# cg-tuwien/StatMC

Hardware: AMD Instinct MI355X
Metric: denoised_mpixels_per_s (higher is better)
Workload: dtype f32

## Files before the change

### include/statmc_debug.h

```cpp
#ifndef STATMC_DEBUG_H
#define STATMC_DEBUG_H

#include "statmc.h"

#include <stddef.h>
#ifdef __cplusplus
extern "C" {
#endif

int statmc_debug_force_filter_variant(int variant);
int statmc_debug_force_filter_parts(int parts);
int statmc_debug_last_filter_parts(void);
int statmc_debug_last_filter_tail(int *parts_hi, int *tail_rows);

int statmc_debug_accumulate_resident_blocks(int n);
int statmc_debug_last_accumulate_grid(void);
int statmc_debug_accumulate_dma(int on);
int statmc_debug_accumulate_launch(int grid_mode, int dma_first);
int statmc_debug_accumulate_umul(int umul);
int statmc_debug_accumulate_tiles_variant(int umul, int order, int wg_per_cu);

int statmc_debug_accumulate_records_phases(int phases);

int statmc_debug_interference_probe(const void *stream_ptr, size_t stream_bytes, void *rmw_ptr, size_t rmw_bytes, float *ms);
int statmc_debug_placement_role(const void *ptr);
float statmc_debug_placement_fast_level(const float *probes_ms, int n, float self_ms);

int statmc_debug_welch_far_items(void);
int statmc_debug_last_workspace(void **ptr, size_t *bytes);

#ifdef __cplusplus
}
#endif
#endif
```

### statmc_amd/api.py

```python
import ctypes as C
import os

from . import build as _build

_HERE = os.path.dirname(os.path.abspath(__file__))

STATMC_OK = 0
ERR_INVALID, ERR_UNSUPPORTED, ERR_HIP, ERR_NO_DEVICE = -1, -2, -3, -4
DOF_PIXEL, DOF_WELCH = 0, 1
MAX_BUFFERS, MAX_GBUFFERS = 16, 8


class StatmcError(RuntimeError):
    def __init__(self, code, msg):
        super().__init__("statmc error %d: %s" % (code, msg))
        self.code = code


class Image(C.Structure):
    _fields_ = [("data", C.c_void_p), ("step", C.c_size_t), ("cols", C.c_int32), ("rows", C.c_int32)]


class FilterArgs(C.Structure):
    _fields_ = [
# ... 107 lines not shown
    lib.statmc_placement_info.argtypes = [C.POINTER(PlacementInfo)]
    lib.statmc_malloc_host.argtypes = [C.POINTER(C.c_void_p), C.c_size_t]
    lib.statmc_free_host.argtypes = [C.c_void_p]
    lib.statmc_memset.argtypes = [C.c_void_p, C.c_int, C.c_size_t, C.c_void_p]
    lib.statmc_upload.argtypes = [C.c_void_p, C.c_void_p, C.c_size_t, C.c_void_p]
    lib.statmc_download.argtypes = [C.c_void_p, C.c_void_p, C.c_size_t, C.c_void_p]
    lib.statmc_stream_create.argtypes = [C.POINTER(C.c_void_p)]
    lib.statmc_stream_create_with_priority.argtypes = [C.POINTER(C.c_void_p), C.c_int]
    lib.statmc_stream_destroy.argtypes = [C.c_void_p]
    lib.statmc_event_create.argtypes = [C.POINTER(C.c_void_p)]
    lib.statmc_event_destroy.argtypes = [C.c_void_p]
    lib.statmc_event_record.argtypes = [C.c_void_p, C.c_void_p]
    lib.statmc_stream_wait_event.argtypes = [C.c_void_p, C.c_void_p]
    lib.statmc_synchronize.argtypes = [C.c_void_p]
    lib.statmc_filter_f32.argtypes = [C.POINTER(FilterArgs)]
    lib.statmc_filter_f32x3.argtypes = [C.POINTER(FilterArgs)]
    lib.statmc_prepass.argtypes = [C.POINTER(FilterArgs), C.c_int]
    lib.statmc_window_filter.argtypes = [C.POINTER(FilterArgs), C.c_int]
    lib.statmc_pack_filter_inputs.argtypes = [C.POINTER(FilterArgs), C.POINTER(Image), C.c_int, C.c_int]
    lib.statmc_prepass_pack.argtypes = [C.POINTER(FilterArgs), C.POINTER(Image), C.c_int, C.c_int]
    lib.statmc_prepass_pack_rows.argtypes = [C.POINTER(FilterArgs), C.POINTER(Image), C.c_int, C.c_int, C.POINTER(C.c_int32), C.c_int]
    lib.statmc_halo_exchange.argtypes = [C.c_void_p, C.c_int, C.c_int, C.c_int, C.c_int, C.c_int]
    lib.statmc_halo_exchange_rccl.argtypes = [C.c_void_p, C.c_int, C.c_int, C.c_int, C.c_int, C.c_int, C.c_void_p, C.c_int]
    lib.statmc_rccl_unique_id.argtypes = [C.c_void_p]
    lib.statmc_rccl_comm_create.argtypes = [C.POINTER(C.c_void_p), C.c_int, C.c_int, C.c_void_p]
    lib.statmc_rccl_comm_destroy.argtypes = [C.c_void_p]
    lib.statmc_copy_rect.argtypes = [C.POINTER(Image), C.c_int, C.c_int, C.c_int, C.POINTER(Image), C.c_int, C.c_int, C.c_int,
                                     C.c_int, C.c_int, C.c_int, C.c_void_p]
    lib.statmc_set_device.argtypes = [C.c_int]
    lib.statmc_calculate_mean_vars.argtypes = [C.c_uint8, C.c_uint16, C.c_uint16, C.c_int,
                                               C.POINTER(Image), C.POINTER(Image), C.POINTER(Image),
                                               C.c_int, C.c_void_p]
    lib.statmc_accumulate.argtypes = [C.c_uint16, C.c_uint16, C.POINTER(StatType), C.c_int, C.c_void_p]
    lib.statmc_accumulate_rows.argtypes = [C.c_uint16, C.c_uint16, C.POINTER(StatType), C.c_int, C.c_int, C.c_int, C.c_void_p]
    lib.statmc_accumulate_row_ranges.argtypes = [C.c_uint16, C.c_uint16, C.POINTER(StatType), C.c_int, C.POINTER(C.c_int32), C.c_int, C.c_void_p]
    lib.statmc_accumulate_tiles.argtypes = [C.c_uint16, C.c_uint16, C.POINTER(StatType), C.c_int, C.c_void_p, C.c_void_p,
                                            C.c_void_p, C.c_int, C.c_void_p]
    lib.statmc_accumulate_records.argtypes = [C.c_uint16, C.c_uint16, C.POINTER(StatType), C.c_int, C.c_void_p, C.c_int64, C.c_void_p]
    lib.statmc_debug_accumulate_records_phases.argtypes = [C.c_int]
    lib.statmc_get_prepass_context.argtypes = [C.POINTER(PrepassContext)]
    lib.statmc_combine_statistics.argtypes = [C.c_uint16, C.c_uint16, C.POINTER(CombineEntry), C.c_int, C.c_void_p]
    lib.statmc_combine_many.argtypes = [C.c_uint16, C.c_uint16, C.POINTER(CombineManyEntry), C.c_int, C.c_int, C.c_void_p]
    lib.statmc_merge_tiles.argtypes = [C.c_uint16, C.c_uint16, C.c_int, C.c_int, C.c_void_p, C.c_void_p,
                                       C.c_void_p, C.c_int, C.c_int] + [C.c_void_p] * 6 + [C.c_void_p]
    lib.statmc_tile_moments.argtypes = [C.c_uint16, C.c_uint16, C.c_int, C.c_void_p, C.c_int,
                                        C.c_void_p, C.c_void_p]
    lib.statmc_film_update.argtypes = [C.c_void_p, C.c_size_t, C.c_float, C.c_float, C.c_void_p, C.c_void_p]
    lib.statmc_clock_probe.argtypes = [C.c_void_p, C.c_int, C.c_void_p]
    lib.statmc_debug_force_filter_variant.argtypes = [C.c_int]
    lib.statmc_debug_force_filter_parts.argtypes = [C.c_int]
    lib.statmc_debug_last_filter_parts.restype = C.c_int
    lib.statmc_debug_accumulate_resident_blocks.argtypes = [C.c_int]
    lib.statmc_debug_accumulate_dma.argtypes = [C.c_int]
    _lib = lib
    return lib


def check(rc):
    if rc != STATMC_OK:
        raise StatmcError(rc, load().statmc_last_error().decode())
    return rc


_setup_done = set()


def setup(device=0):
    if device not in _setup_done:
        check(load().statmc_setup(int(device)))
        _setup_done.add(device)


def set_filter_spec(spec=None, **fields):
    if spec is None and not fields:
        check(load().statmc_reset_filter_spec())
        return
    spec = spec if spec is not None else FilterSpec(**fields)
    check(load().statmc_set_filter_spec(C.byref(spec)))


def get_significance():
    return int(load().statmc_get_significance())


def get_filter_spec():
    spec = FilterSpec()
    check(load().statmc_get_filter_spec(C.byref(spec)))
    return spec


def last_filter_variant():
    return load().statmc_last_filter_variant().decode()


def force_filter_variant(v):
    check(load().statmc_debug_force_filter_variant(int(v)))


def accumulate_resident_blocks(n):
    check(load().statmc_debug_accumulate_resident_blocks(int(n)))


def accumulate_dma(on):
    check(load().statmc_debug_accumulate_dma(int(on)))


def force_filter_parts(k):
    check(load().statmc_set_filter_split(int(k)))


def set_filter_split(parts):
    check(load().statmc_set_filter_split(int(parts)))


def get_filter_split():
    return int(load().statmc_get_filter_split())


def filter_split_auto(width, height, radius):
    k = int(load().statmc_filter_split_auto(int(width), int(height), int(radius)))
    if k < 0:
        check(k)
    return k


def _torch():
    import torch
    return torch


def current_stream_handle():
    return C.c_void_p(_torch().cuda.current_stream().cuda_stream)


def image_of(t):
    assert t.is_cuda and t.element_size() == 4
    h, w = t.shape[0], t.shape[1]
    c = t.shape[2] if t.dim() == 3 else 1
    inner = (t.stride(1) == c and t.stride(2) == 1) if t.dim() == 3 else t.stride(1) == 1
    assert inner and t.stride(0) >= w * c, "device images must have packed pixels and a row pitch of at least one row"
    return Image(C.c_void_p(t.data_ptr()), t.stride(0) * 4, w, h)


def _img_array(tensors):
    arr = (Image * max(len(tensors), 1))()
    for i, t in enumerate(tensors):
        arr[i] = image_of(t)
    return arr


def make_filter_args(n, mean, m2, m3, film, mean_corr, disc, film_filtered, g_buffers, g_sds=None,
                     g_dr=None, filter_sd=10.0, radius=20, denoise_film=False, film_buffer=None,
                     film_filtered_buffer=None, roi=None, stream=None, keep=None, packed=None, film_origin=None,
                     packed_g_channels=None):
    tables = [mean_corr, mean, film, film_filtered, n]
    nb = max(len(t) for t in tables) if packed is None else 1
    ref = next(t[0] for t in tables if t) if packed is None else packed
# ... 315 lines not shown
```

### statmc_amd/csrc/statmc_abi.hip

```cpp

#include <algorithm>
#include <cmath>
#include <stdarg.h>
#include <stdio.h>
#include <string.h>

#include <memory>
#include <mutex>
#include <unordered_map>
#include <vector>

#include "statmc_device.h"

#include <atomic>

#include "t_quantiles.h"
#include "../../include/statmc_pinned_spec.h"

namespace {

thread_local char g_err[512] = "";
thread_local char g_variant[96] = "none";
thread_local int g_last_parts = 0, g_last_parts_hi = 0, g_last_tail_rows = 0;
thread_local const int *g_last_redo = nullptr;
thread_local int g_last_redo_n = 0;
std::mutex g_mu;

struct DeviceState {
    bool ready = false;
    int alpha_index = STATMC_PINNED_SIGNIFICANCE;
    statmc_filter_spec spec = STATMC_PINNED_SPEC;
    int cus = 0;
    int split = 0;
    int force_variant = 0;
    int acc_resident_blocks = 0, acc_umul = 1, acc_dma = 1;
    int acc_grid_mode = -1, acc_dma_first = 0;
    int rec_phases = 3;
    int tiles_umul = 2, tiles_order = 2, tiles_wg_per_cu = 0;
};
std::unordered_map<int, DeviceState> g_dev;

DeviceState current_state(int *dev_out = nullptr) {
    int dev = 0;
    if (hipGetDevice(&dev) != hipSuccess) return DeviceState();
    if (dev_out) *dev_out = dev;
    std::lock_guard<std::mutex> lk(g_mu);
    auto it = g_dev.find(dev);
    return it == g_dev.end() ? DeviceState() : it->second;
}

int fail(int code, const char *fmt, ...) {
    va_list ap;
    va_start(ap, fmt);
    vsnprintf(g_err, sizeof(g_err), fmt, ap);
    va_end(ap);
    return code;
}

}
namespace statmc {
int abi_fail(int code, const char *fmt, ...) {
    va_list ap;
    va_start(ap, fmt);
    vsnprintf(g_err, sizeof(g_err), fmt, ap);
    va_end(ap);
    return code;
}
}
namespace {

#define HIP_TRY(expr)                                                                          \
    do {                                                                                       \
        hipError_t e_ = (expr);                                                                \
        if (e_ != hipSuccess) return fail(STATMC_ERR_HIP, "%s: %s", #expr, hipGetErrorString(e_)); \
    } while (0)

#define NEED_READY()                                                                                      \
    const DeviceState dstate = current_state();                                                           \
    do {                                                                                                  \
        if (!dstate.ready)                                                                                \
            return fail(STATMC_ERR_NO_DEVICE, "statmc_setup() has not been called for the current device"); \
    } while (0)

inline hipStream_t S(void *s) { return reinterpret_cast<hipStream_t>(s); }

struct TabKey {
    int dev, r;
    float ds;
    bool operator==(const TabKey &o) const { return dev == o.dev && r == o.r && memcmp(&ds, &o.ds, 4) == 0; }
// ... 1023 lines not shown
    out->t_table = table;
    out->flags = (dstate.spec.dof == STATMC_DOF_WELCH ? 1 : 0) | (dstate.spec.small_n == STATMC_SMALL_N_EXCLUDE ? 2 : 0);
    out->reserved = 0;
    return STATMC_OK;
}

int statmc_accumulate(uint16_t width, uint16_t height, const statmc_stat_type *types, int n_types, void *stream) {
    return statmc_accumulate_rows(width, height, types, n_types, 0, height, stream);
}
int statmc_accumulate_rows(uint16_t width, uint16_t height, const statmc_stat_type *types, int n_types, int y0, int y1, void *stream) {
    const int32_t range[2] = {y0, y1};
    return statmc_accumulate_row_ranges(width, height, types, n_types, range, 1, stream);
}
int statmc_accumulate_row_ranges(uint16_t width, uint16_t height, const statmc_stat_type *types, int n_types, const int32_t *ranges,
                                 int n_ranges, void *stream) {
    NEED_READY();
    if (width == 0 || height == 0) return fail(STATMC_ERR_INVALID, "empty image");
    if (n_types < 0 || n_ranges < 0 || (long long)n_types * n_ranges > statmc::kMaxStatTypes)
        return fail(STATMC_ERR_INVALID, "stat types x row ranges must be in [0,%d]", statmc::kMaxStatTypes);
    if (n_types == 0 || n_ranges == 0) return STATMC_OK;
    if (!types || !ranges) return fail(STATMC_ERR_INVALID, "null types or ranges");
    statmc::AccumulateArgs k;
    memset(&k, 0, sizeof(k));
    k.n_types = 0;
    for (int r = 0; r < n_ranges; r++) {
        const int y0 = ranges[2 * r], y1 = ranges[2 * r + 1];
        if (y0 < 0 || y1 > height || y0 > y1) return fail(STATMC_ERR_INVALID, "rows [%d,%d) outside the %d-row image", y0, y1, (int)height);
        for (int q = 0; q < r; q++)
            if (y0 < ranges[2 * q + 1] && ranges[2 * q] < y1) return fail(STATMC_ERR_INVALID, "row ranges %d and %d overlap", q, r);
        if (y0 == y1) continue;
        for (int i = 0; i < n_types; i++) {
            statmc::AccumulateType &d = k.t[k.n_types];
            if (int rc = fill_stat_type(dstate, types[i], i, width, height, true, d)) return rc;
            const long long px0 = (long long)y0 * width, e0 = px0 * d.channels;
            if (d.samples) d.samples += e0;
            d.n += px0;
            d.mean += e0;
            if (d.m2) d.m2 += e0;
            if (d.m3) d.m3 += e0;
            if (d.film_mean) d.film_mean += e0;
            if (d.film_m2) d.film_m2 += e0;
            if (d.mean_corr) { d.mean_corr += e0; d.disc += e0; }
            d.n_elems = (long long)(y1 - y0) * width * d.channels;
            k.n_types++;
        }
    }
    if (k.n_types == 0) return STATMC_OK;
    k.resident_blocks = dstate.acc_resident_blocks;
    k.cus = dstate.cus;
    k.umul = dstate.acc_umul;
    k.dma = dstate.acc_dma;
    k.grid_mode = dstate.acc_grid_mode;
    k.dma_first = dstate.acc_dma_first;
    k.occ = 0;
    k.apart = 1;
    for (int i = 0; i < k.n_types && k.apart; i++)
        k.apart = statmc::placement_role_of(k.t[i].samples) == STATMC_MEM_STREAM && statmc::placement_role_of(k.t[i].mean) == STATMC_MEM_STATE;
    HIP_TRY(statmc::launch_accumulate(k, S(stream)));
    return STATMC_OK;
}

static bool aligned16(const void *p) { return (reinterpret_cast<uintptr_t>(p) & 15) == 0; }

static int fill_combine_entry(const DeviceState &ds, const statmc_combine_entry *entries, int n_entries, int i,
                              statmc::CombineEntry &k) {
    const statmc_combine_entry &e = entries[i];
    const statmc_stat_type &d = e.dst, &s = e.src;
    if (d.channels != 1 && d.channels != 3) return fail(STATMC_ERR_INVALID, "entries[%d]: channels must be 1 or 3", i);
    if (d.max_moment < 1 || d.max_moment > 3) return fail(STATMC_ERR_INVALID, "entries[%d]: max_moment must be 1..3", i);
    if (s.channels != d.channels || s.max_moment != d.max_moment)
        return fail(STATMC_ERR_INVALID, "entries[%d]: dst and src disagree on channels or max_moment", i);
    if (e.count_of == -1) {
        if (!d.n || !s.n) return fail(STATMC_ERR_INVALID, "entries[%d]: null n (count_of = -1: the entry's own counts)", i);
        if (d.n == s.n) return fail(STATMC_ERR_INVALID, "entries[%d]: dst.n is src.n", i);
        for (int j = 0; j < i; j++)
            if (entries[j].count_of == -1 && entries[j].dst.n == d.n)
                return fail(STATMC_ERR_INVALID, "entries[%d] and [%d] own the same count image", j, i);
    } else if (e.count_of < 0 || e.count_of >= n_entries || e.count_of == i || entries[e.count_of].count_of != -1) {
        return fail(STATMC_ERR_INVALID, "entries[%d]: bad count_of %d (-1, or an entry with counts of its own)", i, e.count_of);
    } else if (d.n || s.n) {
        return fail(STATMC_ERR_INVALID, "entries[%d]: borrows entry %d's counts, dst.n and src.n must be NULL", i, e.count_of);
    }
    const float *dp[statmc::kCombFields] = {d.mean, d.max_moment >= 2 ? d.m2 : nullptr, d.max_moment >= 3 ? d.m3 : nullptr,
                                            nullptr, nullptr};
    const float *sp[statmc::kCombFields] = {s.mean, s.max_moment >= 2 ? s.m2 : nullptr, s.max_moment >= 3 ? s.m3 : nullptr,
                                            nullptr, nullptr};
    static const char *names[statmc::kCombFields] = {"mean", "m2", "m3", "film_mean", "film_m2"};
    const bool film_mean = d.film_mean && d.film_mean != d.mean;
    const bool film_m2 = d.film_m2 && d.film_m2 != d.m2;
    if (film_m2 && !film_mean) return fail(STATMC_ERR_INVALID, "entries[%d]: film_m2 without a film_mean of its own", i);
    if (film_mean) {
        dp[statmc::kCombFilmMean] = d.film_mean;
        sp[statmc::kCombFilmMean] = s.film_mean;
    }
    if (film_m2) {
        dp[statmc::kCombFilmM2] = d.film_m2;
        sp[statmc::kCombFilmM2] = s.film_m2;
    }
    const int want = d.max_moment;
    for (int f = 0; f < statmc::kCombFields; f++) {
        const bool needed = f < want || (f == statmc::kCombFilmMean && film_mean) || (f == statmc::kCombFilmM2 && film_m2);
        if (!needed) continue;
        if (!dp[f] || !sp[f]) return fail(STATMC_ERR_INVALID, "entries[%d]: null %s", i, names[f]);
        if (dp[f] == sp[f]) return fail(STATMC_ERR_INVALID, "entries[%d]: dst.%s is src.%s", i, names[f], names[f]);
    }
    k.cnt_dst = e.count_of == -1 ? d.n : entries[e.count_of].dst.n;
// ... 229 lines not shown
                              (width + tile_size - 1) / tile_size, (height + tile_size - 1) / tile_size};
    HIP_TRY(statmc::launch_tile_moments(k, S(stream)));
    return STATMC_OK;
}

int statmc_clock_probe(int64_t *out, int cycles, void *stream) {
    NEED_READY();
    if (!out) return fail(STATMC_ERR_INVALID, "null out");
    if (cycles < 1 || cycles > (1 << 24)) return fail(STATMC_ERR_INVALID, "cycles must be in 1 .. 2^24");
    hipLaunchKernelGGL(clock_probe_kernel, dim3(1), dim3(64), 0, S(stream), reinterpret_cast<long long *>(out), (long long)cycles);
    HIP_TRY(hipGetLastError());
    return STATMC_OK;
}

int statmc_set_filter_split(int parts) {
    if (parts < 0 || parts > 64) return fail(STATMC_ERR_INVALID, "parts must be 0 (automatic) .. 64");
    int dev = 0;
    NEED_READY();
    HIP_TRY(hipGetDevice(&dev));
    std::lock_guard<std::mutex> lk(g_mu);
    g_dev[dev].split = parts;
    return STATMC_OK;
}
int statmc_get_filter_split(void) { return current_state().split; }
int statmc_filter_split_auto(int width, int height, int radius) {
    NEED_READY();
    if (width < 1 || height < 1 || radius < 1 || radius > 20) return fail(STATMC_ERR_INVALID, "need a non-empty image and a radius in 1..20");
    statmc::FilterArgs k;
    memset(&k, 0, sizeof(k));
    k.width = width;
    k.height = height;
    k.radius = radius;
    return statmc::whole_image_parts(k, true, dstate.cus, 0);
}

#define STATMC_DEBUG_SET(stmt)                                       \
    do {                                                             \
        int dev = 0;                                                 \
        NEED_READY();                                                \
        HIP_TRY(hipGetDevice(&dev));                                 \
        std::lock_guard<std::mutex> lk(g_mu);                        \
        DeviceState &d = g_dev[dev];                                 \
        stmt;                                                        \
        return STATMC_OK;                                            \
    } while (0)
int statmc_debug_force_filter_variant(int v) {
    if (v < 0 || v > 3) return fail(STATMC_ERR_INVALID, "statmc_debug_force_filter_variant(%d): 0 .. 3", v);
    STATMC_DEBUG_SET(d.force_variant = v);
}
int statmc_debug_accumulate_resident_blocks(int n) {
    STATMC_DEBUG_SET(d.acc_resident_blocks = n < 0 ? -1 : n);
}
int statmc_debug_last_accumulate_grid(void) { return (int)statmc::last_accumulate_grid(); }
int statmc_debug_accumulate_dma(int on) {
    if (on != 0 && on != 1) return fail(STATMC_ERR_INVALID, "statmc_debug_accumulate_dma(%d): 0 or 1", on);
    STATMC_DEBUG_SET(d.acc_dma = on);
}
int statmc_debug_accumulate_launch(int grid_mode, int dma_first) {
    STATMC_DEBUG_SET(d.acc_grid_mode = grid_mode < 0 ? -1 : grid_mode == 1 ? 1 : 0; d.acc_dma_first = dma_first ? 1 : 0);
}
int statmc_debug_accumulate_umul(int umul) {
    STATMC_DEBUG_SET(d.acc_umul = umul == 2 ? 2 : 1);
}
int statmc_debug_accumulate_tiles_variant(int umul, int order, int wg_per_cu) {
    STATMC_DEBUG_SET(d.tiles_umul = umul == 2 ? 2 : 1; d.tiles_order = order < 0 || order > 2 ? 0 : order; d.tiles_wg_per_cu = wg_per_cu < 0 ? 0 : wg_per_cu);
}
int statmc_debug_accumulate_records_phases(int phases) {
    if (phases < 1 || phases > 3) return fail(STATMC_ERR_INVALID, "statmc_debug_accumulate_records_phases(%d): 1, 2 or 3", phases);
    STATMC_DEBUG_SET(d.rec_phases = phases);
}
int statmc_debug_force_filter_parts(int k) { return statmc_set_filter_split(k < 0 ? 0 : k); }
int statmc_debug_last_filter_parts(void) { return g_last_parts; }
int statmc_debug_last_filter_tail(int *parts_hi, int *tail_rows) {
    if (parts_hi) *parts_hi = g_last_parts_hi;
    if (tail_rows) *tail_rows = g_last_tail_rows;
    return STATMC_OK;
}
int statmc_debug_welch_far_items(void) {
    if (g_last_redo == nullptr || g_last_redo_n <= 0) return -1;
    if (hipDeviceSynchronize() != hipSuccess) return -1;
    std::vector<int> f((size_t)g_last_redo_n);
    if (hipMemcpy(f.data(), g_last_redo, f.size() * sizeof(int), hipMemcpyDeviceToHost) != hipSuccess) return -1;
    int n = 0;
    for (int v : f) n += v != 0;
    return n;
}
int statmc_debug_last_workspace(void **ptr, size_t *bytes) {
    int dev = 0;
    HIP_TRY(hipGetDevice(&dev));
    std::lock_guard<std::mutex> lk(g_mu);
    *ptr = nullptr;
    *bytes = 0;
    for (auto &kv : g_ws)
        if (kv.first.dev == dev && kv.second.bytes > *bytes) {
            *ptr = kv.second.ptr;
            *bytes = kv.second.bytes;
        }
    return STATMC_OK;
}
}
```

### statmc_amd/csrc/statmc_device.h

```cpp
#pragma once

#include <hip/hip_runtime.h>
#include <stdint.h>

#include "../../include/statmc.h"

namespace statmc {

struct PrepassArgs {
    const int32_t *n;
    const float *mean, *m2, *m3;
    float *mean_corr, *disc;
    long long n_elems;
    int channels;
    int table;
    int welch;
    int small_n_exclude;
};

struct MeanVarsArgs {
    const int32_t *n;
    const float *film_m2;
    float *film_var;
    int width, height, channels, row_n_quirk;
};

constexpr int kMaxStatTypes = 16;
struct AccumulateType {
    const float *samples;
    int32_t *n;
    float *mean, *m2, *m3, *film_mean, *film_m2;
    long long n_elems;
    long long stride;
    int channels, n_samples, transform, max_moment;
    float *mean_corr, *disc;
    int pre_table;
    int pre_flags;
};
constexpr int kMaxSlots = 64;
struct AccumulateArgs {
    AccumulateType t[kMaxStatTypes];
    int n_types;
    int resident_blocks;
    int cus;
    int umul;
    int dma;
    int grid_mode;
    int dma_first;
    int occ;
    int apart;
    int n_slots;
    int type_slots[kMaxStatTypes];
    unsigned char slot_type[kMaxSlots], slot_rank[kMaxSlots];
};

struct AccumulateTilesArgs {
    AccumulateType t[kMaxStatTypes];
    int n_types;
    const int32_t *tile_bounds;
    const long long *tile_offsets;
    const int32_t *tile_samples;
    int n_tiles, width, height, vec;
    int dma;
    int umul, order, wg_per_cu;
    int dma_first;
};

enum { kCombMean = 0, kCombM2, kCombM3, kCombFilmMean, kCombFilmM2, kCombFields };
struct CombineEntry {
    int32_t *cnt_dst;
    const int32_t *cnt_src;
    float *d[kCombFields];
    const float *s[kCombFields];
    float *mean_corr, *disc;
    int channels, write_n, pre_table, pre_flags;
};
struct CombineArgs {
    CombineEntry e[kMaxStatTypes];
    int n_entries;
    int vec;
    long long n_px;
};
hipError_t launch_combine(const CombineArgs &a, hipStream_t s);

enum { kCombManyPlanes = 3, kCombManySrcPtrs = 1 + kCombManyPlanes, kCombManySlots = 90 };
struct CombineManyEntry {
    int32_t *cnt_dst;
    float *d[kCombManyPlanes];
    float *mean_corr, *disc;
    int channels, moments, write_n, pre;
};
struct CombineManyArgs {
    long long n_px;
    int n_entries, n_sources;
    int vec;
    int reserved;
    CombineManyEntry e[kMaxStatTypes];
    const void *src[kCombManySlots * kCombManySrcPtrs];
};
static_assert(sizeof(CombineManyArgs) <= 4096, "CombineManyArgs is passed by value: the kernel-argument limit");
hipError_t launch_combine_many(const CombineManyArgs &a, hipStream_t s);

struct RecordsArgs {
    statmc_stat_type t[kMaxStatTypes];
    statmc_prepass_context ctx;
    const int32_t *order;
// ... 58 lines not shown
    const int32_t *f_n[3];
    float *f_out[3];
    int f_active;
    const float *packed;
    int packed_ch;
    struct SymGeom {
        int tx0, ty0, ntx, nty;
        int fx0, fy0;
        long long item_stride4;
        float4 *patch;
        int pair;
        float *pair_images;
        float4 *border_extra;
        int *redo;
        int parts_hi, split_ty, n_lo_tiles, n_lo_items;
        int steps;
        const float *tab_rt;
        int g8;
        const float *rgb[2], *sc[2];
        float rgb_scale[2], sc_scale[2];
    } sym;
};

struct PackArgs {
    const float *mean_corr, *disc, *colour, *g0, *g1;
    float *packed;
    int src_w, src_h, dst_w, dst_x0, dst_y0;
    const float *s0, *s1;
    int ch;
    const int32_t *n;
};
hipError_t launch_pack_inputs(const PackArgs &a, hipStream_t s);

struct PrepassPackArgs {
    const int32_t *n;
    const float *mean, *m2, *m3, *colour, *g0, *g1;
    float *mean_corr, *disc;
    float *packed;
    int src_w, src_h, dst_w, dst_x0, dst_y0, table, welch, small_n_exclude;
    int split_row, skip_rows;
    const float *s0, *s1;
    int ch;
};
hipError_t launch_prepass_pack(const PrepassPackArgs &a, hipStream_t s);

hipError_t upload_t_tables();
hipError_t upload_t_table(int table, const float *host_4096);
const float *t_table_device_ptr(int table);
const float *t_table_sq_device_ptr(int table);
hipError_t launch_prepass(const PrepassArgs &a, hipStream_t s);
hipError_t launch_mean_vars(const MeanVarsArgs &a, hipStream_t s);
hipError_t launch_accumulate(const AccumulateArgs &a, hipStream_t s);
unsigned last_accumulate_grid();
hipError_t launch_accumulate_tiles(const AccumulateTilesArgs &a, hipStream_t s);
hipError_t launch_merge_tiles(const MergeTilesArgs &a, int n_tiles, int max_tile_pixels, hipStream_t s);
hipError_t launch_tile_moments(const TileMomentsArgs &a, hipStream_t s);
hipError_t launch_film_update(const void *pixels, long long n, float splat_scale, float scale, float *rgb, hipStream_t s);

enum { kFilterGeneric, kFilterLds, kFilterSym };
struct FilterPlan {
    int kernel;
    bool lds_r20;
    int per_launch;
    bool lds_tail;
    bool spatial_tab, sym_rt_tab;
    size_t partial_floats, patch_floats, image_floats, extra_floats, redo_floats;
    int redo_items;
    int tail_rows;
    char variant[48], tail_variant[96];
};
int plan_window_filter(FilterArgs &k, int channels, int n_buffers, int n_cus, int force_variant, int split, FilterPlan &p);
hipError_t launch_window_filter(const FilterPlan &p, bool tail, const FilterArgs &a, int channels, hipStream_t s);
int whole_image_parts(const FilterArgs &a, bool sym, int n_cus, int split);
size_t spatial_table_floats(int radius);
size_t sym_rt_table_floats(int radius);
void fill_sym_rt_table(float *host_tab, int radius, float ds);
void fill_spatial_table(float *host_tab, int radius, float ds);

int abi_fail(int code, const char *fmt, ...);
int placement_role_of(const void *ptr);
int placement_free(void *ptr);
hipError_t workspace_alloc(void **p, size_t bytes);
hipError_t workspace_free(void *p);
hipError_t placement_grant_peer(int owner_device, int peer_device);

}
```

### statmc_amd/csrc/statmc_pointwise.hip

```cpp

#include <type_traits>

#include "statmc_device.h"

#include "../../include/statmc_device_api.hpp"
#include "t_quantiles.h"

namespace statmc {

using device::CombineCounts;
using device::ElemState;
using device::add_sample;
using device::div_by_count;
using device::prepass_elem;
using device::refined_rcp;

constexpr int kAccURgbT = 3, kAccURgb = 3, kAccUF = 6;
constexpr int kAccPairGroup = 3;
constexpr int kAccWaves = 2;
constexpr int kAccDmaD = 3;
constexpr int kAccTilesDmaD = 3;
constexpr int acc_ring_floats(int d) { return d * 3 * 256; }
constexpr size_t acc_lds_bytes(int d) { return (size_t)4 * acc_ring_floats(d) * sizeof(float); }
template <int N> __device__ __forceinline__ void acc_wait_vmcnt() { asm volatile("s_waitcnt vmcnt(%0)" ::"n"(N) : "memory"); }
// ... 447 lines not shown
        const int n_active = left >= 64 ? 64 : left > 0 ? (int)left : 0;
        if (n_active > 0)
            accumulate_lane<C, MAXM, TRANSFORM, (!TRANSFORM && MAXM == 1) ? UMUL : 1, DMA>(t, p0, t.samples + p0 * C, t.stride, t.n_samples,
                                                                                            ring, active, n_active, dma_first);
        if (!active && g < n_groups) {
            for (long long p = p0; p < n_px && p < p0 + 4; p++)
                accumulate_pixel<C, MAXM, TRANSFORM>(t, p, t.samples + p * C, t.stride, t.n_samples);
        }
    }
}

template <int C, bool VEC, int UMUL, int DMA>
__device__ __forceinline__ void accumulate_dispatch(const AccumulateType &t, long long blk, long long nblk, float *ring, bool dma_first) {
    if (t.transform) {
        if (t.max_moment >= 3) accumulate_type<C, 3, true, VEC, UMUL, DMA>(t, blk, nblk, ring, dma_first);
        else if (t.max_moment == 2) accumulate_type<C, 2, true, VEC, UMUL, DMA>(t, blk, nblk, ring, dma_first);
        else accumulate_type<C, 1, true, VEC, UMUL, DMA>(t, blk, nblk, ring, dma_first);
    } else {
        if (t.max_moment >= 3) accumulate_type<C, 3, false, VEC, UMUL, DMA>(t, blk, nblk, ring, dma_first);
        else if (t.max_moment == 2) accumulate_type<C, 2, false, VEC, UMUL, DMA>(t, blk, nblk, ring, dma_first);
        else accumulate_type<C, 1, false, VEC, UMUL, DMA>(t, blk, nblk, ring, dma_first);
    }
}

template <bool VEC, int UMUL, int DMA, int OCC = kAccWaves>
__global__ __launch_bounds__(kBlock, OCC) void accumulate_kernel(AccumulateArgs a) {
    extern __shared__ __attribute__((aligned(16))) float acc_lds[];
    float *ring = DMA ? acc_lds + (threadIdx.x >> 6) * acc_ring_floats(DMA) : nullptr;
    if (a.resident_blocks > 0) {
        for (int i = 0; i < a.n_types; i++) {
            const AccumulateType t = a.t[((int)blockIdx.x + i) % a.n_types];
            if (t.channels == 3) accumulate_dispatch<3, VEC, UMUL, DMA>(t, blockIdx.x, gridDim.x, ring, a.dma_first != 0);
            else accumulate_dispatch<1, VEC, UMUL, DMA>(t, blockIdx.x, gridDim.x, ring, a.dma_first != 0);
        }
        return;
    }
    if (a.grid_mode == 1) {
        const int ti = blockIdx.x % a.n_types;
        const AccumulateType t = a.t[ti];
        const long long blk = blockIdx.x / a.n_types, nblk = gridDim.x / a.n_types;
        if (t.channels == 3) accumulate_dispatch<3, VEC, UMUL, DMA>(t, blk, nblk, ring, a.dma_first != 0);
        else accumulate_dispatch<1, VEC, UMUL, DMA>(t, blk, nblk, ring, a.dma_first != 0);
        return;
    }
    const int slot = blockIdx.x % a.n_slots, round = blockIdx.x / a.n_slots, n_rounds = gridDim.x / a.n_slots;
    const int ti = a.slot_type[slot];
    const AccumulateType t = a.t[ti];
    const long long blk = (long long)round * a.type_slots[ti] + a.slot_rank[slot];
    const long long nblk = (long long)n_rounds * a.type_slots[ti];
    if (t.channels == 3) accumulate_dispatch<3, VEC, UMUL, DMA>(t, blk, nblk, ring, a.dma_first != 0);
    else accumulate_dispatch<1, VEC, UMUL, DMA>(t, blk, nblk, ring, a.dma_first != 0);
}

static thread_local unsigned g_last_acc_grid = 0;
unsigned last_accumulate_grid() { return g_last_acc_grid; }

hipError_t launch_accumulate(const AccumulateArgs &a_in, hipStream_t s) {
    AccumulateArgs a = a_in;
    a.n_slots = 0;
    for (int i = 0; i < a.n_types; i++) {
        int w = a.t[i].channels * (a.t[i].transform ? 4 : 3);
        w = (w + 2) / 3;
        if (w < 1) w = 1;
        a.type_slots[i] = w;
        for (int r = 0; r < w && a.n_slots < kMaxSlots; r++) {
            a.slot_type[a.n_slots] = (unsigned char)i;
            a.slot_rank[a.n_slots] = (unsigned char)r;
            a.n_slots++;
        }
    }
    {
        unsigned char st[kMaxSlots], sr[kMaxSlots];
        int n = 0;
        for (int r = 0; n < a.n_slots; r++)
            for (int i = 0; i < a.n_types; i++)
                if (r < a.type_slots[i]) { st[n] = (unsigned char)i; sr[n] = (unsigned char)r; n++; }
        for (int k = 0; k < a.n_slots; k++) { a.slot_type[k] = st[k]; a.slot_rank[k] = sr[k]; }
    }
    bool vec = true;
    long long max_groups = 1;
    for (int i = 0; i < a.n_types; i++) {
        const AccumulateType &t = a.t[i];
        vec = vec && aligned16(t.samples) && aligned16(t.n) && aligned16(t.mean) &&
              (t.max_moment < 2 || aligned16(t.m2)) && (t.max_moment < 3 || aligned16(t.m3)) &&
              (!t.transform || (aligned16(t.film_mean) && aligned16(t.film_m2))) &&
              (!t.mean_corr || (aligned16(t.mean_corr) && aligned16(t.disc))) &&
              (t.n_elems % 4 == 0) && (t.stride % 4 == 0);
        const long long groups = (t.n_elems / t.channels + 3) / 4;
        if (groups > max_groups) max_groups = groups;
    }
    const int rounds = (grid_for(max_groups, 256 * 8) * a.n_types + a.n_slots - 1) / a.n_slots;
    const long long units = (max_groups + kBlock - 1) / kBlock;
    int max_s = 0;
    for (int i = 0; i < a.n_types; i++) max_s = a.t[i].n_samples > max_s ? a.t[i].n_samples : max_s;
    if (a.resident_blocks == 0 && a.grid_mode < 0 && a.apart && a.cus > 0 && max_s >= 256 && max_groups >= (1 << 18) && max_groups < 3 * (1 << 18)) {
        const double walks = (double)max_groups / ((double)a.cus * kBlock);
        if (walks / ceil(walks) >= 0.97) a.resident_blocks = a.cus;
    }
    if (a.resident_blocks < 0) a.resident_blocks = 0;
    if (a.grid_mode < 0) {
        const bool big = max_groups >= (1 << 20);
        if (a.apart) a.grid_mode = (max_s <= 16 || big || max_s >= 128) ? 1 : 0;
        else a.grid_mode = (max_s <= 8 || (max_s <= 16 && !big)) ? 1 : 0;
    }
    const dim3 grid(a.resident_blocks > 0 ? a.resident_blocks : a.grid_mode == 1 ? (unsigned)(units * a.n_types) : rounds * a.n_slots);
    g_last_acc_grid = grid.x;
    if (vec && a.dma) {
        hipLaunchKernelGGL((accumulate_kernel<true, 1, kAccDmaD>), grid, dim3(kBlock), acc_lds_bytes(kAccDmaD), s, a);
        return hipGetLastError();
    }
    if (vec && a.umul == 2)
        hipLaunchKernelGGL((accumulate_kernel<true, 2, 0>), grid, dim3(kBlock), 0, s, a);
    else if (vec)
        hipLaunchKernelGGL((accumulate_kernel<true, 1, 0>), grid, dim3(kBlock), 0, s, a);
    else
        hipLaunchKernelGGL((accumulate_kernel<false, 1, 0>), grid, dim3(kBlock), 0, s, a);
    return hipGetLastError();
}

template <int C, int MAXM, bool TRANSFORM, int UMUL, int DMA>
__device__ __forceinline__ void accumulate_tile(const AccumulateType &t, const AccumulateTilesArgs &a, int x0, int y0,
                                                int tw, int th, long long off, int S, float *ring) {
    const int lane = threadIdx.x & 63;
    const int npx = tw * th;
    const float *base = t.samples + off * C;
    const long long stride = (long long)npx * C;
    const bool fast = a.vec && ((tw | x0 | a.width) & 3) == 0 && (off & 3) == 0;
    if (fast) {
        const int n_g = npx >> 2;
        for (int gw = 0; gw < n_g; gw += 64) {
            const int g = gw + lane;
            const bool active = g < n_g;
            const int i = g << 2, row = i / tw, col = i - row * tw;
            const long long p0 = (long long)(y0 + row) * a.width + x0 + col;
            accumulate_lane<C, MAXM, TRANSFORM, (!TRANSFORM && MAXM == 1) ? UMUL : 1, DMA>(t, p0, base + (long long)i * C, stride, S, ring, active,
                                                                                            n_g - gw >= 64 ? 64 : n_g - gw, a.dma_first != 0);
        }
    } else {
        for (int i = lane; i < npx; i += 64) {
            const int row = i / tw, col = i - row * tw;
            const long long p = (long long)(y0 + row) * a.width + x0 + col;
            accumulate_pixel<C, MAXM, TRANSFORM>(t, p, base + (long long)i * C, stride, S);
        }
    }
}

template <int C, int UMUL, int DMA>
__device__ __forceinline__ void accumulate_tile_dispatch(const AccumulateType &t, const AccumulateTilesArgs &a, int x0,
                                                         int y0, int tw, int th, long long off, int S, float *ring) {
    if (t.transform) {
        if (t.max_moment >= 3) accumulate_tile<C, 3, true, UMUL, DMA>(t, a, x0, y0, tw, th, off, S, ring);
        else if (t.max_moment == 2) accumulate_tile<C, 2, true, UMUL, DMA>(t, a, x0, y0, tw, th, off, S, ring);
// ... 479 lines not shown
```

Baseline: 388.5.

## Fuse radiance and feature-buffer accumulation into one persistent LDS-ring kernel

Adds a fused accumulate kernel that walks the radiance type and up to two RGB and two scalar feature types in one wave loop. It streams samples of all types into a shared LDS ring via global_load_lds with counted vmcnt waits, and keeps per-pixel state in registers across samples. Waves whose per-pixel counts differ fall back to a ragged per-type path. The kernel is launched with one block per CU when the shape heuristic matches (many samples, mid-size images) or when forced. It aims to cut per-type launch and slot overhead and overlap loads across types, at the cost of a large LDS footprint, single-block occupancy and high register pressure.

Result: faster. 393.4, median of 6 (+1.3%).

```diff
diff --git a/include/statmc_debug.h b/include/statmc_debug.h
--- a/include/statmc_debug.h
+++ b/include/statmc_debug.h
@@ -15,6 +15,8 @@
 
 int statmc_debug_accumulate_resident_blocks(int n);
 int statmc_debug_last_accumulate_grid(void);
+int statmc_debug_accumulate_fused(int mode);
+int statmc_debug_last_accumulate_fused(void);
 int statmc_debug_accumulate_dma(int on);
 int statmc_debug_accumulate_launch(int grid_mode, int dma_first);
 int statmc_debug_accumulate_umul(int umul);
diff --git a/statmc_amd/api.py b/statmc_amd/api.py
--- a/statmc_amd/api.py
+++ b/statmc_amd/api.py
@@ -183,6 +183,8 @@
     lib.statmc_debug_last_filter_parts.restype = C.c_int
     lib.statmc_debug_accumulate_resident_blocks.argtypes = [C.c_int]
     lib.statmc_debug_accumulate_dma.argtypes = [C.c_int]
+    lib.statmc_debug_accumulate_fused.argtypes = [C.c_int]
+    lib.statmc_debug_last_accumulate_fused.restype = C.c_int
     _lib = lib
     return lib
 
@@ -234,6 +236,14 @@
 
 def accumulate_dma(on):
     check(load().statmc_debug_accumulate_dma(int(on)))
+
+
+def accumulate_fused(mode):
+    check(load().statmc_debug_accumulate_fused(int(mode)))
+
+
+def last_accumulate_fused():
+    return int(load().statmc_debug_last_accumulate_fused())
 
 
 def force_filter_parts(k):
diff --git a/statmc_amd/csrc/statmc_abi.hip b/statmc_amd/csrc/statmc_abi.hip
--- a/statmc_amd/csrc/statmc_abi.hip
+++ b/statmc_amd/csrc/statmc_abi.hip
@@ -35,6 +35,7 @@
     int force_variant = 0;
     int acc_resident_blocks = 0, acc_umul = 1, acc_dma = 1;
     int acc_grid_mode = -1, acc_dma_first = 0;
+    int acc_fused = 0;
     int rec_phases = 3;
     int tiles_umul = 2, tiles_order = 2, tiles_wg_per_cu = 0;
 };
@@ -1164,6 +1165,7 @@
     k.dma = dstate.acc_dma;
     k.grid_mode = dstate.acc_grid_mode;
     k.dma_first = dstate.acc_dma_first;
+    k.fused = dstate.acc_fused;
     k.occ = 0;
     k.apart = 1;
     for (int i = 0; i < k.n_types && k.apart; i++)
@@ -1499,6 +1501,11 @@
     STATMC_DEBUG_SET(d.acc_resident_blocks = n < 0 ? -1 : n);
 }
 int statmc_debug_last_accumulate_grid(void) { return (int)statmc::last_accumulate_grid(); }
+int statmc_debug_accumulate_fused(int mode) {
+    if (mode < -1 || mode > 1) return fail(STATMC_ERR_INVALID, "statmc_debug_accumulate_fused(%d): -1, 0 or 1", mode);
+    STATMC_DEBUG_SET(d.acc_fused = mode);
+}
+int statmc_debug_last_accumulate_fused(void) { return statmc::last_accumulate_fused(); }
 int statmc_debug_accumulate_dma(int on) {
     if (on != 0 && on != 1) return fail(STATMC_ERR_INVALID, "statmc_debug_accumulate_dma(%d): 0 or 1", on);
     STATMC_DEBUG_SET(d.acc_dma = on);
diff --git a/statmc_amd/csrc/statmc_device.h b/statmc_amd/csrc/statmc_device.h
--- a/statmc_amd/csrc/statmc_device.h
+++ b/statmc_amd/csrc/statmc_device.h
@@ -52,6 +52,7 @@
     int n_slots;
     int type_slots[kMaxStatTypes];
     unsigned char slot_type[kMaxSlots], slot_rank[kMaxSlots];
+    int fused;
 };
 
 struct AccumulateTilesArgs {
@@ -216,6 +217,7 @@
 hipError_t launch_mean_vars(const MeanVarsArgs &a, hipStream_t s);
 hipError_t launch_accumulate(const AccumulateArgs &a, hipStream_t s);
 unsigned last_accumulate_grid();
+int last_accumulate_fused();
 hipError_t launch_accumulate_tiles(const AccumulateTilesArgs &a, hipStream_t s);
 hipError_t launch_merge_tiles(const MergeTilesArgs &a, int n_tiles, int max_tile_pixels, hipStream_t s);
 hipError_t launch_tile_moments(const TileMomentsArgs &a, hipStream_t s);
diff --git a/statmc_amd/csrc/statmc_pointwise.hip b/statmc_amd/csrc/statmc_pointwise.hip
--- a/statmc_amd/csrc/statmc_pointwise.hip
+++ b/statmc_amd/csrc/statmc_pointwise.hip
@@ -523,8 +523,320 @@
     else accumulate_dispatch<1, VEC, UMUL, DMA>(t, blk, nblk, ring, a.dma_first != 0);
 }
 
+#ifndef STATMC_ACC_FUSED_D
+#define STATMC_ACC_FUSED_D 3
+#endif
+constexpr int kAccFusedD = STATMC_ACC_FUSED_D;
+constexpr int kAccFusedTypes = 5;
+struct AccumulateFusedArgs {
+    AccumulateType t[kAccFusedTypes];
+    long long n_groups;
+    int n_samples;
+};
+constexpr int acc_fused_slot_floats(int k, int m) { return 768 * (1 + k) + 256 * m; }
+constexpr size_t acc_fused_lds_bytes(int k, int m, int d) { return (size_t)4 * d * acc_fused_slot_floats(k, m) * sizeof(float); }
+
+template <int K, int M, int D>
+__device__ __forceinline__ void accumulate_fused_ragged(const AccumulateFusedArgs &a, long long gw, int n_active, float *ring) {
+    static_assert(K >= 0 && K <= 2 && M >= 0 && M <= 2, "a.t[1] / a.t[K] and a.t[1 + K] / a.t[K + M] name every feature type only up to two of a kind");
+    constexpr int kFit = D * acc_fused_slot_floats(K, M) / 768;
+    constexpr int FD = kFit < kAccDmaD ? kFit : kAccDmaD;
+    const int lane = threadIdx.x & 63;
+    const long long p0 = (gw + lane) << 2;
+    const bool active = lane < n_active;
+    const int S = a.n_samples;
+    {
+        const AccumulateType t = a.t[0];
+        accumulate_lane<3, 3, true, 1, FD>(t, p0, t.samples + p0 * 3, t.stride, S, ring, active, n_active, false);
+    }
+    if constexpr (K > 0) {
+#pragma unroll 1
+        for (int i = 0; i < K; i++) {
+            const AccumulateType t = i == 0 ? a.t[1] : a.t[K];
+            accumulate_lane<3, 1, false, 1, FD>(t, p0, t.samples + p0 * 3, t.stride, S, ring, active, n_active, false);
+        }
+    }
+    if constexpr (M > 0) {
+#pragma unroll 1
+        for (int i = 0; i < M; i++) {
+            const AccumulateType t = i == 0 ? a.t[1 + K] : a.t[K + M];
+            accumulate_lane<1, 1, false, 1, FD>(t, p0, t.samples + p0, t.stride, S, ring, active, n_active, false);
+        }
+    }
+}
+
+template <int K, int M, int D>
+__device__ __forceinline__ void accumulate_fused_wave(const AccumulateFusedArgs &a, long long gw, int n_active, float *ring) {
+    constexpr int NT = 1 + K + M;
+    constexpr int SLOT = acc_fused_slot_floats(K, M);
+    constexpr int T = 3 * (1 + K) + M;
+    static_assert(T * (D - 1) <= 63, "the counted wait must fit vmcnt");
+    constexpr int KA = K > 0 ? K : 1, MA = M > 0 ? M : 1;
+    const int lane = threadIdx.x & 63;
+    const bool active = lane < n_active;
+    const long long p0 = active ? (gw + lane) << 2 : 0;
+    const int S = a.n_samples;
+    int nb[NT];
+    bool lane_same = true, lane_one = true;
+#pragma unroll
+    for (int i = 0; i < NT; i++) {
+        const int4 n4 = *reinterpret_cast<const int4 *>(a.t[i].n + p0);
+        nb[i] = n4.x;
+        lane_same = lane_same && n4.x == n4.y && n4.y == n4.z && n4.z == n4.w;
+        lane_one = lane_one && n4.x == nb[0];
+    }
+    if (__builtin_amdgcn_ballot_w64(active && !lane_same) != 0) {
+        accumulate_fused_ragged<K, M, D>(a, gw, n_active, ring);
+        return;
+    }
+    float *const r_mean = a.t[0].mean, *const r_m2 = a.t[0].m2, *const r_m3 = a.t[0].m3, *const r_fmean = a.t[0].film_mean,
+                 *const r_fm2 = a.t[0].film_m2, *const pre_mc = a.t[0].mean_corr, *const pre_dc = a.t[0].disc;
+    const int pre_table = a.t[0].pre_table, pre_flags = a.t[0].pre_flags;
+    int32_t *n_ptr[NT];
+    float *f_mean[NT];
+    const float *row[NT];
+    long long stride[NT];
+#pragma unroll
+    for (int i = 0; i < NT; i++) {
+        n_ptr[i] = a.t[i].n;
+        f_mean[i] = a.t[i].mean;
+        row[i] = a.t[i].samples + (gw << 2) * (i <= K ? 3 : 1);
+        stride[i] = a.t[i].stride;
+    }
+    int piece3[3];
+#pragma unroll
+    for (int k = 0; k < 3; k++) piece3[k] = 256 * k + 4 * lane < 12 * n_active ? 256 * k + 4 * lane : 0;
+    const int piece1 = active ? 4 * lane : 0;
+    auto issue = [&](int slot) {
+        float *dst = ring + slot * SLOT;
+#pragma unroll
+        for (int i = 0; i < NT; i++) {
+            if (i <= K) {
+#pragma unroll
+                for (int k = 0; k < 3; k++)
+                    __builtin_amdgcn_global_load_lds(row[i] + piece3[k], (__attribute__((address_space(3))) void *)(dst + 768 * i + 256 * k), 16, 0, 2);
+            } else {
+                __builtin_amdgcn_global_load_lds(row[i] + piece1, (__attribute__((address_space(3))) void *)(dst + 768 * (1 + K) + 256 * (i - 1 - K)), 16, 0, 2);
+            }
+            row[i] += stride[i];
+        }
+    };
+    const long long e3 = p0 * 3;
+    PairState st[6], fr[KA][6], f1[MA][2];
+    auto load3 = [&](const float *p, v2f (&d)[6]) {
+#pragma unroll
+        for (int k = 0; k < 3; k++) {
+            const float4 v = *reinterpret_cast<const float4 *>(p + e3 + 4 * k);
+            d[2 * k] = v2f{v.x, v.y};
+            d[2 * k + 1] = v2f{v.z, v.w};
+        }
+    };
+    {
+        v2f d[6];
+#define STATMC_FUSED_LOAD(ptr, arr, field) load3(ptr, d); _Pragma("unroll") for (int j = 0; j < 6; j++) arr[j].field = d[j];
+        STATMC_FUSED_LOAD(r_mean, st, mean)
+        STATMC_FUSED_LOAD(r_m2, st, m2)
+        STATMC_FUSED_LOAD(r_m3, st, m3)
+        STATMC_FUSED_LOAD(r_fmean, st, fmean)
+        STATMC_FUSED_LOAD(r_fm2, st, fm2)
+#pragma unroll
+        for (int i = 0; i < K; i++) { STATMC_FUSED_LOAD(f_mean[1 + i], fr[i], mean) }
+#undef STATMC_FUSED_LOAD
+#pragma unroll
+        for (int i = 0; i < M; i++) {
+            const float4 v = *reinterpret_cast<const float4 *>(f_mean[1 + K + i] + p0);
+            f1[i][0].mean = v2f{v.x, v.y};
+            f1[i][1].mean = v2f{v.z, v.w};
+        }
+    }
+    auto walk = [&](auto one) {
+        acc_wait_vmcnt<0>();
+#pragma unroll
+        for (int d = 0; d < D; d++)
+            if (d < S) issue(d);
+        const int S_full = S >= D ? S - D + 1 : 0;
+        int slot = 0;
+#pragma unroll 1
+        for (int s = 0; s < S; s++) {
+            if (s < S_full) acc_wait_vmcnt<T * (D - 1)>(); else acc_wait_vmcnt<0>();
+            const float *mine = ring + slot * SLOT;
+            vfloat4 q[1 + K][3], q1[MA];
+#pragma unroll
+            for (int i = 0; i <= K; i++)
+#pragma unroll
+                for (int k = 0; k < 3; k++) q[i][k] = *reinterpret_cast<const vfloat4 *>(mine + 768 * i + 12 * lane + 4 * k);
+#pragma unroll
+            for (int i = 0; i < M; i++) q1[i] = *reinterpret_cast<const vfloat4 *>(mine + 768 * (1 + K) + 256 * i + 4 * lane);
+            asm volatile("s_waitcnt lgkmcnt(0)" ::: "memory");
+            if (s + D < S) issue(slot);
+            v2f nf[NT], rc[NT];
+            if constexpr (decltype(one)::value) {
+                const float nf0 = (float)(nb[0] + s + 1);
+                const float rc0 = refined_rcp(nf0);
+#pragma unroll
+                for (int i = 0; i < NT; i++) { nf[i] = v2f{nf0, nf0}; rc[i] = v2f{rc0, rc0}; }
+            } else {
+#pragma unroll
+                for (int i = 0; i < NT; i++) {
+                    const float nfi = (float)(nb[i] + s + 1);
+                    const float rci = refined_rcp(nfi);
+                    nf[i] = v2f{nfi, nfi};
+                    rc[i] = v2f{rci, rci};
+                }
+            }
+#pragma unroll
+            for (int i = 0; i < M; i++) {
+                const v2f nf2[2] = {nf[1 + K + i], nf[1 + K + i]}, rc2[2] = {rc[1 + K + i], rc[1 + K + i]};
+                const v2f smp2[2] = {v2f{q1[i][0], q1[i][1]}, v2f{q1[i][2], q1[i][3]}};
+                add_sample2<2, 1, false>(f1[i], nf2, rc2, smp2);
+            }
+            auto fold3 = [&](PairState *state, int i, auto radiance) {
+                const v2f nf3[3] = {nf[i], nf[i], nf[i]}, rc3[3] = {rc[i], rc[i], rc[i]};
+                v2f smp2[6];
+#pragma unroll
+                for (int j = 0; j < 6; j++) smp2[j] = v2f{q[i][j >> 1][2 * (j & 1)], q[i][j >> 1][2 * (j & 1) + 1]};
+#pragma unroll
+                for (int g = 0; g < 6; g += kAccPairGroup) {
+                    if constexpr (decltype(radiance)::value) add_sample2<kAccPairGroup, 3, true>(state + g, nf3, rc3, smp2 + g);
+                    else add_sample2<kAccPairGroup, 1, false>(state + g, nf3, rc3, smp2 + g);
+                }
+            };
+#pragma unroll
+            for (int i = 0; i < K; i++) fold3(fr[i], 1 + i, std::false_type{});
+            fold3(st, 0, std::true_type{});
+            slot = slot + 1 == D ? 0 : slot + 1;
+        }
+    };
+    if (__builtin_amdgcn_ballot_w64(active && !lane_one) == 0) walk(std::true_type{});
+    else walk(std::false_type{});
+    if (!active) return;
+    auto store3 = [&](float *p, const v2f (&d)[6]) {
+#pragma unroll
+        for (int k = 0; k < 3; k++) {
+            const vfloat4 v = {d[2 * k].x, d[2 * k].y, d[2 * k + 1].x, d[2 * k + 1].y};
+            *reinterpret_cast<vfloat4 *>(p + e3 + 4 * k) = v;
+        }
+    };
+    {
+        v2f d[6];
+#define STATMC_FUSED_STORE(ptr, arr, field) _Pragma("unroll") for (int j = 0; j < 6; j++) d[j] = arr[j].field; store3(ptr, d);
+        STATMC_FUSED_STORE(r_mean, st, mean)
+        STATMC_FUSED_STORE(r_m2, st, m2)
+        STATMC_FUSED_STORE(r_m3, st, m3)
+        STATMC_FUSED_STORE(r_fmean, st, fmean)
+        STATMC_FUSED_STORE(r_fm2, st, fm2)
+#pragma unroll
+        for (int i = 0; i < K; i++) { STATMC_FUSED_STORE(f_mean[1 + i], fr[i], mean) }
+#undef STATMC_FUSED_STORE
+#pragma unroll
+        for (int i = 0; i < M; i++) {
+            const vfloat4 v = {f1[i][0].mean.x, f1[i][0].mean.y, f1[i][1].mean.x, f1[i][1].mean.y};
+            *reinterpret_cast<vfloat4 *>(f_mean[1 + K + i] + p0) = v;
+        }
+    }
+    typedef int vint4 __attribute__((ext_vector_type(4)));
+#pragma unroll
+    for (int i = 0; i < NT; i++) {
+        const vint4 n_out = {nb[i] + S, nb[i] + S, nb[i] + S, nb[i] + S};
+        *reinterpret_cast<vint4 *>(n_ptr[i] + p0) = n_out;
+    }
+    if (pre_mc != nullptr) {
+        const int n_out = nb[0] + S;
+        const float tq = (pre_flags & 1) ? 1.f : t_quantile(pre_table, n_out - 1);
+#pragma unroll
+        for (int k = 0; k < 3; k++) {
+            vfloat4 mc, dc;
+#pragma unroll
+            for (int j = 0; j < 4; j++) {
+                const int e = 4 * k + j;
+                float m, d;
+                prepass_elem(n_out, tq, st[e >> 1].mean[e & 1], st[e >> 1].m2[e & 1], st[e >> 1].m3[e & 1], m, d, (pre_flags & 2) != 0);
+                mc[j] = m;
+                dc[j] = d;
+            }
+            *reinterpret_cast<vfloat4 *>(pre_mc + e3 + 4 * k) = mc;
+            *reinterpret_cast<vfloat4 *>(pre_dc + e3 + 4 * k) = dc;
+        }
+    }
+}
+
+template <int K, int M, int D>
+__global__ __launch_bounds__(kBlock, 1) void accumulate_fused_kernel(AccumulateFusedArgs a) {
+    extern __shared__ __attribute__((aligned(16))) float acc_lds[];
+    const int wave = __builtin_amdgcn_readfirstlane(threadIdx.x >> 6);
+    float *ring = acc_lds + wave * (D * acc_fused_slot_floats(K, M));
+    for (long long gw = (long long)blockIdx.x * kBlock + wave * 64; gw < a.n_groups; gw += (long long)gridDim.x * kBlock) {
+        const long long left = a.n_groups - gw;
+        accumulate_fused_wave<K, M, D>(a, gw, left >= 64 ? 64 : (int)left, ring);
+    }
+}
+
+static bool accumulate_fused_plan(const AccumulateArgs &a, AccumulateFusedArgs &f, int &K, int &M) {
+    K = M = 0;
+    if (a.n_types < 2 || a.n_types > kAccFusedTypes) return false;
+    const long long n_px = a.t[0].n_elems / a.t[0].channels;
+    const int S = a.t[0].n_samples;
+    if (S < 1 || n_px < 4 || n_px % 4 != 0) return false;
+    int rad = -1, rgb[2] = {0, 0}, f1[2] = {0, 0};
+    for (int i = 0; i < a.n_types; i++) {
+        const AccumulateType &t = a.t[i];
+        if (t.n_elems / t.channels != n_px || t.n_samples != S) return false;
+        if (t.channels == 3 && t.transform && t.max_moment >= 3) {
+            if (rad >= 0) return false;
+            rad = i;
+        } else if (!t.transform && t.max_moment == 1 && t.channels == 3) {
+            if (K == 2) return false;
+            rgb[K++] = i;
+        } else if (!t.transform && t.max_moment == 1 && t.channels == 1) {
+            if (M == 2) return false;
+            f1[M++] = i;
+        } else {
+            return false;
+        }
+    }
+    if (rad < 0 || K + M < 1) return false;
+    f = AccumulateFusedArgs{};
+    f.t[0] = a.t[rad];
+    for (int i = 0; i < K; i++) f.t[1 + i] = a.t[rgb[i]];
+    for (int i = 0; i < M; i++) f.t[1 + K + i] = a.t[f1[i]];
+    f.n_groups = n_px / 4;
+    f.n_samples = S;
+    return true;
+}
+
+template <int K, int M>
+static hipError_t launch_accumulate_fused_km(const AccumulateFusedArgs &f, unsigned blocks, hipStream_t s) {
+    constexpr size_t lds = acc_fused_lds_bytes(K, M, kAccFusedD);
+    const void *fn = reinterpret_cast<const void *>(&accumulate_fused_kernel<K, M, kAccFusedD>);
+    static thread_local unsigned long long allowed = 0;
+    int dev = 0;
+    if (hipError_t e = hipGetDevice(&dev); e != hipSuccess) return e;
+    if (dev < 0 || dev >= 64 || !((allowed >> dev) & 1)) {
+        if (hipError_t e = hipFuncSetAttribute(fn, hipFuncAttributeMaxDynamicSharedMemorySize, (int)lds); e != hipSuccess) return e;
+        if (dev >= 0 && dev < 64) allowed |= 1ull << dev;
+    }
+    hipLaunchKernelGGL((accumulate_fused_kernel<K, M, kAccFusedD>), dim3(blocks), dim3(kBlock), lds, s, f);
+    return hipGetLastError();
+}
+
+static hipError_t launch_accumulate_fused(const AccumulateFusedArgs &f, int K, int M, unsigned blocks, hipStream_t s) {
+    switch (3 * K + M) {
+    case 1: return launch_accumulate_fused_km<0, 1>(f, blocks, s);
+    case 2: return launch_accumulate_fused_km<0, 2>(f, blocks, s);
+    case 3: return launch_accumulate_fused_km<1, 0>(f, blocks, s);
+    case 4: return launch_accumulate_fused_km<1, 1>(f, blocks, s);
+    case 5: return launch_accumulate_fused_km<1, 2>(f, blocks, s);
+    case 6: return launch_accumulate_fused_km<2, 0>(f, blocks, s);
+    case 7: return launch_accumulate_fused_km<2, 1>(f, blocks, s);
+    case 8: return launch_accumulate_fused_km<2, 2>(f, blocks, s);
+    }
+    return hipErrorInvalidValue;
+}
+
 static thread_local unsigned g_last_acc_grid = 0;
+static thread_local int g_last_acc_fused = 0;
 unsigned last_accumulate_grid() { return g_last_acc_grid; }
+int last_accumulate_fused() { return g_last_acc_fused; }
 
 hipError_t launch_accumulate(const AccumulateArgs &a_in, hipStream_t s) {
     AccumulateArgs a = a_in;
@@ -564,11 +876,26 @@
     const long long units = (max_groups + kBlock - 1) / kBlock;
     int max_s = 0;
     for (int i = 0; i < a.n_types; i++) max_s = a.t[i].n_samples > max_s ? a.t[i].n_samples : max_s;
+    const int resident_asked = a.resident_blocks;
     if (a.resident_blocks == 0 && a.grid_mode < 0 && a.apart && a.cus > 0 && max_s >= 256 && max_groups >= (1 << 18) && max_groups < 3 * (1 << 18)) {
         const double walks = (double)max_groups / ((double)a.cus * kBlock);
         if (walks / ceil(walks) >= 0.97) a.resident_blocks = a.cus;
     }
     if (a.resident_blocks < 0) a.resident_blocks = 0;
+    g_last_acc_fused = 0;
+    if (a.fused >= 0 && resident_asked >= 0 && vec && a.dma) {
+        const bool by_shape = a.fused == 0 && resident_asked == 0 && a.grid_mode < 0 && a.cus > 0 &&
+                              (a.resident_blocks > 0 || (max_s >= 128 && max_groups >= 128000 && max_groups < (1 << 19)));
+        AccumulateFusedArgs f;
+        int K = 0, M = 0;
+        if ((by_shape || a.fused == 1) && accumulate_fused_plan(a, f, K, M)) {
+            const long long most = a.cus > 0 && a.cus < units ? a.cus : units;
+            const unsigned blocks = resident_asked > 0 ? (unsigned)resident_asked : a.resident_blocks > 0 ? (unsigned)a.resident_blocks : (unsigned)most;
+            g_last_acc_grid = blocks;
+            g_last_acc_fused = 1;
+            return launch_accumulate_fused(f, K, M, blocks, s);
+        }
+    }
     if (a.grid_mode < 0) {
         const bool big = max_groups >= (1 << 20);
         if (a.apart) a.grid_mode = (max_s <= 16 || big || max_s >= 128) ? 1 : 0;
```
